# nivihelen99/NetFlow

Measured on AMD Instinct MI355X. Metric: device-resident payload GB/s checksummed, batched packets, 1/2/4/8 MI355X, higher is better.
Workload: dtype u16 one's-complement (u8 frames, u32 word sums); 1 GPU; C1: 1M x 1500 B IPv4+UDP, device-resident; packets_per_gpu=1048576, frame_align=128, frame_bytes_per_gpu=1572864000, parallelism=independent shards x1

## Files before the change

### netflow_amd/csrc/nfcs_api.hip

```cpp
#include <pthread.h>
#include <sched.h>
#include <stdio.h>
#include <stdlib.h>
#include <string.h>
#include <sys/mman.h>
#include <sys/syscall.h>
#include <unistd.h>

#include <algorithm>
#include <chrono>
#include <condition_variable>
#include <mutex>
#include <new>
#include <thread>
#include <type_traits>
#include <vector>

#include "nfcs_internal.h"
#include "nfcs_store_policy.h"

struct HostBlock {
    void* p = nullptr;
    size_t bytes = 0;
    bool mapped = false;
// ... 111 lines not shown
    nfcs_patch* h_patch[kSlots] = {nullptr, nullptr};
    uint64_t* d_digest = nullptr;
    hipEvent_t ev0 = nullptr, ev1 = nullptr;
    nfcs_patch* ws = nullptr;
    size_t ws_cap = 0;
    hipEvent_t ws_ev = nullptr;
    hipStream_t ws_stream = nullptr;
    bool ws_used = false;
    bool ws_own = false;
    uint32_t* eq_ws = nullptr;
    uint64_t eq_cap = 0;
    hipEvent_t eq_ev = nullptr;
    hipStream_t eq_stream = nullptr;
    bool eq_used = false;
    bool eq_own = false;
    uint32_t slot_bytes = 0;
    static constexpr int kObsSlots = 8;
    uint64_t* obs_host = nullptr;
    uint64_t* obs_dev = nullptr;
    struct ObsBurst { const void* desc; uint32_t n; uint64_t bytes; uint32_t gen; uint64_t used; };
    ObsBurst obs_burst[kObsSlots] = {};
    uint32_t obs_gen = 0;
    uint64_t obs_clock = 0;
    static constexpr int kDemRing = 64;
    uint32_t* dem_dev = nullptr;
    uint64_t* dem_host = nullptr;
    uint64_t* dem_host_dev = nullptr;
    uint32_t dem_gen = 0;
    struct DemCall { uint32_t gen, sampled; };
    DemCall dem_calls[kDemRing] = {};
// ... 68 lines not shown
            (void)hipGetLastError();
            return hipErrorOutOfMemory;
        }
        c->eq_cap = cap;
    } else if (c->eq_used && c->eq_stream != st) {
        hipError_t e = wait_eq_user(c, st);
        if (e != hipSuccess) return e;
    }
    return hipSuccess;
}
hipError_t release_eq(nfcs_ctx* c, hipStream_t st) {
    c->eq_stream = st;
    c->eq_used = true;
    c->eq_own = st == c->stream;
    return c->eq_own ? hipSuccess : hipEventRecord(c->eq_ev, st);
}

int hip_fail(hipError_t e) {
    g_last_hip = (int)e;
    return NFCS_EHIP;
}
#define NFCS_HIP(x)                              \
    do {                                         \
        hipError_t e_ = (x);                     \
        if (e_ != hipSuccess) return hip_fail(e_); \
    } while (0)

hipStream_t pick(nfcs_ctx* ctx, void* s) { return s ? (hipStream_t)s : ctx->stream; }

struct DeviceGuard {
// ... 617 lines not shown
}

template <class Launch>
int with_eq_scratch(nfcs_ctx* c, uint64_t words, hipStream_t st, Launch&& launch) {
    const hipError_t e = acquire_eq(c, words, st);
    if (e == hipErrorOutOfMemory) {
        (void)hipGetLastError();
        return NFCS_ENOMEM;
    }
    NFCS_HIP(e);
    NFCS_HIP(launch(c->eq_ws));
    NFCS_HIP(release_eq(c, st));
    return NFCS_OK;
}

}

extern "C" {

NFCS_API int nfcs_abi_version(void) { return NFCS_ABI_VERSION; }

NFCS_API const char* nfcs_strerror(int err) {
    switch (err) {
    case NFCS_OK: return "ok";
    case NFCS_EINVAL: return "invalid argument";
    case NFCS_EHIP: return "HIP runtime error";
    case NFCS_ENOMEM: return "out of memory";
    case NFCS_ENODEV: return "no gfx950 device";
    default: return "unknown error";
    }
// ... 11 lines not shown
    }
    DeviceGuard dg_(device);
    if (dg_.err != hipSuccess) return hip_fail(dg_.err);
    hipDeviceProp_t prop;
    NFCS_HIP(hipGetDeviceProperties(&prop, device));
    if (strncmp(prop.gcnArchName, "gfx950", 6) != 0) return NFCS_ENODEV;
    nfcs_ctx* c = new (std::nothrow) nfcs_ctx();
    if (!c) return NFCS_ENOMEM;
    c->di.device = device;
    c->di.cus = prop.multiProcessorCount;
    strncpy(c->di.arch, prop.gcnArchName, sizeof(c->di.arch) - 1);
    hipError_t e = hipStreamCreateWithFlags(&c->stream, hipStreamNonBlocking);
    if (e == hipSuccess) e = hipMalloc(&c->d_digest, sizeof(uint64_t));
    if (e == hipSuccess) e = hipEventCreateWithFlags(&c->ws_ev, hipEventDisableTiming);
    if (e == hipSuccess) e = hipEventCreateWithFlags(&c->eq_ev, hipEventDisableTiming);
    if (e == hipSuccess) e = hipEventCreate(&c->ev0);
    if (e == hipSuccess) e = hipEventCreate(&c->ev1);
    if (e == hipSuccess) e = hipHostMalloc((void**)&c->obs_host, nfcs_ctx::kObsSlots * sizeof(uint64_t), hipHostMallocMapped);
    if (e == hipSuccess) {
        for (int k = 0; k < nfcs_ctx::kObsSlots; ++k) c->obs_host[k] = 0;
        e = hipHostGetDevicePointer((void**)&c->obs_dev, c->obs_host, 0);
    }
    const size_t dem_bytes = 2u * nfcs::kDemandWords * nfcs::kDemandStrideWords * sizeof(uint32_t);
    if (e == hipSuccess) e = hipMalloc((void**)&c->dem_dev, dem_bytes);
    if (e == hipSuccess) e = hipMemset(c->dem_dev, 0, dem_bytes);
    if (e == hipSuccess) e = hipHostMalloc((void**)&c->dem_host, sizeof(uint64_t), hipHostMallocMapped);
    if (e == hipSuccess) {
        *c->dem_host = 0;
        e = hipHostGetDevicePointer((void**)&c->dem_host_dev, c->dem_host, 0);
    }
    if (e != hipSuccess) {
        nfcs_ctx_destroy(c);
        return hip_fail(e);
    }
    *out = c;
    return NFCS_OK;
}

NFCS_API int nfcs_ctx_destroy(nfcs_ctx* c) {
    if (!c) return NFCS_OK;
    DeviceGuard dg_(c->di.device);
    if (c->stream) (void)hipStreamSynchronize(c->stream);
    if (c->ws_used && !c->ws_own && c->ws_ev) (void)hipEventSynchronize(c->ws_ev);
    if (c->eq_used && !c->eq_own && c->eq_ev) (void)hipEventSynchronize(c->eq_ev);
    free_host_pipeline(c);
    if (c->d_digest) (void)hipFree(c->d_digest);
    if (c->eq_ws) (void)hipFree(c->eq_ws);
    if (c->eq_ev) (void)hipEventDestroy(c->eq_ev);
    if (c->ws) (void)hipFree(c->ws);
    if (c->ws_ev) (void)hipEventDestroy(c->ws_ev);
    if (c->ev0) (void)hipEventDestroy(c->ev0);
    if (c->ev1) (void)hipEventDestroy(c->ev1);
    if (c->stream) (void)hipStreamDestroy(c->stream);
    if (c->obs_host) (void)hipHostFree(c->obs_host);
    if (c->dem_host) (void)hipHostFree(c->dem_host);
    if (c->dem_dev) (void)hipFree(c->dem_dev);
    delete c;
    return NFCS_OK;
}

NFCS_API void* nfcs_ctx_stream(nfcs_ctx* c) { return c ? (void*)c->stream : nullptr; }

NFCS_API int nfcs_ctx_set_slot_bytes(nfcs_ctx* c, uint32_t bytes) {
// ... 635 lines not shown
}

NFCS_API int nfcs_egress_acl_device(nfcs_ctx* c, const nfcs_aclset* s, const uint8_t* d_arena, uint64_t arena_bytes,
                                    const nfcs_desc* d_desc, uint32_t n, uint32_t* d_port, uint8_t* d_action,
                                    uint32_t* d_rule, uint32_t* d_redirect, uint32_t* d_denied_pkts,
                                    uint64_t* d_denied_bytes, void* stream) {
    if (!usable(c, s)) return NFCS_EINVAL;
    if (!d_denied_pkts != !d_denied_bytes) return NFCS_EINVAL;
    DeviceGuard dg_(c->di.device);
    if (dg_.err != hipSuccess) return hip_fail(dg_.err);
    if (n == 0) return NFCS_OK;
    if (!d_arena || !d_desc || !d_port || !d_action || ((uintptr_t)d_arena & 15u)) return NFCS_EINVAL;
    if (((uintptr_t)d_port & 3u) || ((uintptr_t)d_rule & 3u) || ((uintptr_t)d_redirect & 3u) ||
        ((uintptr_t)d_denied_pkts & 3u) || ((uintptr_t)d_denied_bytes & 7u))
        return NFCS_EINVAL;
    NFCS_HIP(nfcs::launch_egress_acl(c->di, s->dev, d_arena, arena_bytes, d_desc, n, d_port, d_action, d_rule, d_redirect,
                                     d_denied_pkts, d_denied_bytes, pick(c, stream)));
    return NFCS_OK;
}

}

struct nfcs_txq {
    nfcs::TxqTables t;
    nfcs::TxqState h;
    nfcs_ctx* ctx = nullptr;
    int device = -1;
    uint8_t* d_blob = nullptr;
    uint8_t* d_ring = nullptr;
    size_t state_off = 0, state_bytes = 0;
    nfcs::TxqDev dev;
};

// ... 241 lines not shown
                                          uint32_t n, const uint8_t* d_action, const uint32_t* d_redirect,
                                          const uint8_t* d_rt_verdict, uint32_t* d_nh, uint32_t* d_l2_port,
                                          uint8_t* d_l2_verdict, uint8_t* d_class, uint8_t* d_bypass,
                                          nfcs_rx_stats* d_rx_stats, void* stream) {
    if (!usable(c, f)) return NFCS_EINVAL;
    DeviceGuard dg_(c->di.device);
    if (dg_.err != hipSuccess) return hip_fail(dg_.err);
    if (n == 0) return NFCS_OK;
    if (!d_arena || !d_desc || !d_rt_verdict || !d_nh || !d_l2_port || !d_l2_verdict || ((uintptr_t)d_arena & 15u))
        return NFCS_EINVAL;
    if (((uintptr_t)d_redirect & 3u) || ((uintptr_t)d_nh & 3u) || ((uintptr_t)d_l2_port & 3u) ||
        ((uintptr_t)d_rx_stats & 7u))
        return NFCS_EINVAL;
    const nfcs::DispatchArgs a{d_arena, arena_bytes, ingress_port, num_ports, n, d_desc, d_action, d_redirect,
                               d_rt_verdict, d_nh, d_l2_port, d_l2_verdict, d_class, d_bypass, d_rx_stats};
    NFCS_HIP(nfcs::launch_ingress_dispatch(c->di, f->dev, a, pick(c, stream)));
    return NFCS_OK;
}

NFCS_API int nfcs_egress_acl_items_host(const nfcs_aclset* s, const uint8_t* arena, uint64_t arena_bytes,
                                        const nfcs_desc* desc, uint32_t n, uint32_t* port, const uint32_t* item_src,
                                        const uint8_t* bypass, uint32_t n_src, uint8_t* action, uint32_t* rule,
                                        uint32_t* redirect, uint32_t* denied_pkts, uint64_t* denied_bytes) {
    if (!s || !s->committed || (!denied_pkts != !denied_bytes) || (!item_src != !bypass)) return NFCS_EINVAL;
    if (n == 0) return NFCS_OK;
    if (!arena || !desc || !port || !action) return NFCS_EINVAL;
    nfcs::aclset_egress(s->t, arena, arena_bytes, desc, n, port, action, rule, redirect, denied_pkts, denied_bytes,
                        item_src, bypass, n_src);
    return NFCS_OK;
}

NFCS_API int nfcs_egress_acl_items_device(nfcs_ctx* c, const nfcs_aclset* s, const uint8_t* d_arena, uint64_t arena_bytes,
                                          const nfcs_desc* d_desc, uint32_t n, uint32_t* d_port,
                                          const uint32_t* d_item_src, const uint8_t* d_bypass, uint32_t n_src,
                                          uint8_t* d_action, uint32_t* d_rule, uint32_t* d_redirect,
                                          uint32_t* d_denied_pkts, uint64_t* d_denied_bytes, void* stream) {
    if (!usable(c, s)) return NFCS_EINVAL;
    if ((!d_denied_pkts != !d_denied_bytes) || (!d_item_src != !d_bypass)) return NFCS_EINVAL;
    DeviceGuard dg_(c->di.device);
    if (dg_.err != hipSuccess) return hip_fail(dg_.err);
    if (n == 0) return NFCS_OK;
    if (!d_arena || !d_desc || !d_port || !d_action || ((uintptr_t)d_arena & 15u)) return NFCS_EINVAL;
    if (((uintptr_t)d_port & 3u) || ((uintptr_t)d_rule & 3u) || ((uintptr_t)d_redirect & 3u) ||
        ((uintptr_t)d_denied_pkts & 3u) || ((uintptr_t)d_denied_bytes & 7u) || ((uintptr_t)d_item_src & 3u))
        return NFCS_EINVAL;
    NFCS_HIP(nfcs::launch_egress_acl(c->di, s->dev, d_arena, arena_bytes, d_desc, n, d_port, d_action, d_rule, d_redirect,
                                     d_denied_pkts, d_denied_bytes, pick(c, stream), d_item_src, d_bypass, n_src));
    return NFCS_OK;
}

}

namespace {
struct RxWorkspace {
    uint64_t nh, eif, red, l2p, iport, ops, vlan, rt, st, act, l2v, byp, queue, eact, total;
};
RxWorkspace rx_workspace(uint32_t n, uint32_t cap) {
    uint64_t at = 0;
    auto part = [&at](uint64_t bytes) {
        const uint64_t o = at;
        at += (bytes + 15u) & ~15ull;
        return o;
    };
// ... 33 lines not shown
    if (!io->d_key_start || (tb->egress->dev.keys > 0 && !io->d_depth)) return NFCS_EINVAL;
    if (((uintptr_t)io->d_item_desc & 7u) || ((uintptr_t)io->d_item_port & 3u) || ((uintptr_t)io->d_item_src & 3u) ||
        ((uintptr_t)io->d_order & 3u) || ((uintptr_t)io->d_key_start & 3u) || ((uintptr_t)io->d_key_dropped & 3u) ||
        ((uintptr_t)io->d_depth & 3u) || ((uintptr_t)io->d_denied_pkts & 3u) || ((uintptr_t)io->d_denied_bytes & 7u) ||
        ((uintptr_t)io->d_rx_stats & 7u))
        return NFCS_EINVAL;
    hipStream_t st = pick(c, stream);
    uint8_t* ws = (uint8_t*)io->d_workspace;
    uint32_t *d_nh = (uint32_t*)(ws + w.nh), *d_eif = (uint32_t*)(ws + w.eif), *d_red = (uint32_t*)(ws + w.red);
    uint32_t *d_l2p = (uint32_t*)(ws + w.l2p), *d_iport = (uint32_t*)(ws + w.iport), *d_ops = (uint32_t*)(ws + w.ops);
    uint16_t* d_vlan = (uint16_t*)(ws + w.vlan);
    uint8_t *d_rt = ws + w.rt, *d_st = ws + w.st, *d_act = ws + w.act, *d_l2v = ws + w.l2v, *d_byp = ws + w.byp;
    uint8_t *d_queue = ws + w.queue, *d_eact = ws + w.eact;
    const bool acl = tb->ingress_acl != nullptr;
    const uint64_t frames = io->copy_base;
    NFCS_HIP(nfcs::launch_route_lookup(c->di, tb->fib->dev, io->d_arena, frames, io->d_desc, n, d_nh, d_eif, d_rt, st));
    if (acl)
        NFCS_HIP(nfcs::launch_acl_eval(c->di, tb->ingress_acl->dev, io->d_arena, frames, io->d_desc, n, d_act, nullptr,
                                       d_red, d_nh, st));
    NFCS_HIP(nfcs::launch_l2_lookup(c->di, tb->fdb->dev, io->ingress_port, io->d_arena, frames, io->d_desc, n, d_rt, d_l2p,
                                    d_l2v, d_vlan, nullptr, st));
    const nfcs::DispatchArgs da{io->d_arena, frames, io->ingress_port, io->num_ports, n, io->d_desc,
                                acl ? d_act : nullptr, acl ? d_red : nullptr, d_rt, d_nh, d_l2p, d_l2v, io->d_class, d_byp,
                                io->d_rx_stats};
    NFCS_HIP(nfcs::launch_ingress_dispatch(c->di, tb->fdb->dev, da, st));
    int rc = l3_forward_device(c, io->d_arena, frames, io->d_desc, d_nh, n, tb->fib->d_table, tb->fib->d_table_n, d_st, st);
    if (rc != NFCS_OK) return rc;
    const nfcs::FloodArgs fa{io->d_arena, io->arena_bytes, io->copy_base, io->copy_align, io->ingress_port, io->num_ports,
                             n, cap, io->d_desc, d_eif, d_st, d_l2p, d_l2v, d_vlan, io->d_item_desc, d_iport,
                             io->d_item_src, io->d_totals};
    rc = with_eq_scratch(c, nfcs::flood_scratch_words(n), st, [&](uint32_t* sc) {
        return nfcs::launch_flood_expand(c->di, tb->fdb->dev, fa, sc, st);
    });
    if (rc != NFCS_OK || cap == 0) return rc;
    NFCS_HIP(nfcs::launch_egress_plan(c->di, tb->egress->dev, io->d_arena, io->arena_bytes, io->d_item_desc, cap, nullptr,
                                      nullptr, d_iport, io->d_item_port, d_ops, d_queue, st));
    {
        const Shape sh = launch_shape(c, io->arena_bytes, io->d_item_desc, cap, kVlanRule);
        NFCS_HIP(nfcs::launch_vlan(c->di, io->d_arena, io->arena_bytes, io->d_item_desc, cap, d_ops, 0u, nullptr, 0u, nullptr,
                                   st, sh.mean, sh.obs, sh.bits));
    }
    if (tb->aclset)
        NFCS_HIP(nfcs::launch_egress_acl(c->di, tb->aclset->dev, io->d_arena, io->arena_bytes, io->d_item_desc, cap,
                                         io->d_item_port, d_eact, nullptr, nullptr, io->d_denied_pkts, io->d_denied_bytes,
                                         st, io->d_item_src, d_byp, n));
    rc = with_eq_scratch(c, nfcs::egress_scratch_words(cap, tb->egress->dev.keys), st, [&](uint32_t* sc) {
        return nfcs::launch_egress_enqueue(c->di, tb->egress->dev, io->d_item_port, d_queue, cap, io->d_depth, nullptr,
                                           io->d_order, io->d_key_start, io->d_key_dropped, sc, st);
    });
    if (rc != NFCS_OK) return rc;
    if (tb->txq)
        NFCS_HIP(nfcs::launch_txq_append(tb->txq->dev, io->d_order, io->d_key_start, io->d_depth, nullptr, nullptr, cap, st,
                                         io->handle_base));
    return NFCS_OK;
}

NFCS_API int nfcs_update_host(nfcs_ctx* c, uint8_t* h_arena, uint64_t arena_bytes,
                              const nfcs_desc* h_desc, uint32_t n, uint8_t* h_status,
                              uint32_t flags) {
    if (!c) return NFCS_EINVAL;
// ... 357 lines not shown
    if (!d_arena || !d_desc) return NFCS_EINVAL;
    NFCS_HIP(nfcs::launch_stale_every(d_arena, arena_bytes, d_desc, n, every, pick(c, stream)));
    return NFCS_OK;
}

NFCS_API int nfcs_digest_device(nfcs_ctx* c, const uint8_t* d_arena, uint64_t arena_bytes,
                                const nfcs_desc* d_desc, uint32_t n, uint64_t first,
                                uint64_t* h_digest, void* stream) {
    if (!c || !h_digest) return NFCS_EINVAL;
    DeviceGuard dg_(c->di.device);
    if (dg_.err != hipSuccess) return hip_fail(dg_.err);
    hipStream_t st = pick(c, stream);
    NFCS_HIP(hipMemsetAsync(c->d_digest, 0, sizeof(uint64_t), st));
    if (n) {
        if (!d_arena || !d_desc) return NFCS_EINVAL;
        NFCS_HIP(nfcs::launch_digest(c->di, d_arena, arena_bytes, d_desc, n, first, c->d_digest, st));
    }
    NFCS_HIP(hipMemcpyAsync(h_digest, c->d_digest, sizeof(uint64_t), hipMemcpyDeviceToHost, st));
    NFCS_HIP(hipStreamSynchronize(st));
    return NFCS_OK;
}

NFCS_API int nfcs_device_alloc(nfcs_ctx* c, size_t bytes, void** out) {
    if (!c || !out) return NFCS_EINVAL;
    DeviceGuard dg_(c->di.device);
    if (dg_.err != hipSuccess) return hip_fail(dg_.err);
    hipError_t e = hipMalloc(out, bytes ? bytes : 16);
    if (e == hipErrorOutOfMemory) { (void)hipGetLastError(); return NFCS_ENOMEM; }
    NFCS_HIP(e);
    return NFCS_OK;
}
// ... 178 lines not shown
```

### netflow_amd/csrc/nfcs_internal.h

```cpp
#pragma once

#include <hip/hip_runtime.h>
#include <stdint.h>

#include "nfcs.h"
#include "nfcs_acl.h"
#include "nfcs_aclset.h"
#include "nfcs_egress.h"
#include "nfcs_fdb.h"
#include "nfcs_fib.h"
#include "nfcs_icmp.h"
#include "nfcs_switch.h"
#include "nfcs_txq.h"

namespace nfcs {

constexpr int kWave = 64;
constexpr int kWavesPerBlock = 4;
constexpr int kBlock = kWave * kWavesPerBlock;

struct DevInfo {
    int device = 0;
    int cus = 256;
    char arch[64] = {0};
// ... 47 lines not shown
struct DemandReq {
    uint32_t* cur = nullptr;
    uint32_t* prev = nullptr;
    uint64_t* host = nullptr;
    uint32_t prev_gen = 0;
};
constexpr uint32_t kDemandSampleEvery = 64;
constexpr uint32_t kDemandWords = 64, kDemandStrideWords = 32;
constexpr uint32_t kDemandBlockPackets = 16;
inline uint32_t demand_sampled_one(uint32_t n) {
    const uint32_t span = kDemandSampleEvery * kDemandBlockPackets;
    const uint32_t rest = n % span;
    return n / span * kDemandBlockPackets + (rest < kDemandBlockPackets ? rest : kDemandBlockPackets);
}

hipError_t launch_update(const DevInfo& di, uint8_t* arena, uint64_t arena_bytes,
                         const nfcs_desc* desc, uint32_t n, uint32_t base16, uint8_t* status,
                         nfcs_patch* patch, nfcs_patch* ws, int form, hipStream_t stream,
                         uint64_t slot_bytes = 0, ObsReq obs = {}, DoneReq done = {}, DemandReq dem = {},
                         bool sparse = false);
uint32_t update_demand_sampled(uint64_t arena_bytes, uint32_t n, uint64_t slot_bytes, bool sparse);

hipError_t launch_l3_forward(const DevInfo& di, uint8_t* arena, uint64_t arena_bytes,
                             const nfcs_desc* desc, const uint32_t* nh, uint32_t n,
                             const nfcs_nexthop* table, uint32_t table_n, uint8_t* status,
                             nfcs_patch* ws, hipStream_t stream, uint64_t slot_bytes = 0,
                             ObsReq obs = {});

hipError_t launch_vlan(const DevInfo& di, uint8_t* arena, uint64_t arena_bytes, nfcs_desc* desc,
                       uint32_t n, const uint32_t* ops, uint32_t op_all, const uint32_t* caps,
// ... 26 lines not shown
};

hipError_t launch_acl_eval(const DevInfo& di, const AclDev& acl, const uint8_t* arena, uint64_t arena_bytes,
                           const nfcs_desc* desc, uint32_t n, uint8_t* action, uint32_t* rule, uint32_t* redirect,
                           uint32_t* nh, hipStream_t stream);

struct AclSetDev {
    const uint4* rec = nullptr;
    const uint2* act = nullptr;
    const uint2* bind = nullptr;
    uint32_t ports = 0, rules_padded = 0;
};

hipError_t launch_egress_acl(const DevInfo& di, const AclSetDev& set, const uint8_t* arena, uint64_t arena_bytes,
                             const nfcs_desc* desc, uint32_t n, uint32_t* port, uint8_t* action, uint32_t* rule,
                             uint32_t* redirect, uint32_t* denied_pkts, uint64_t* denied_bytes, hipStream_t stream,
                             const uint32_t* item_src = nullptr, const uint8_t* bypass = nullptr, uint32_t n_src = 0);

struct FdbDev {
    const uint4* slots = nullptr;
    uint32_t slot_mask = 0, max_probe = 0;
    const uint8_t* port_state = nullptr;
    const uint16_t* port_native = nullptr;
    const uint32_t* port_vlans = nullptr;
    uint32_t ports = 0;
    const uint32_t* vlan_ports = nullptr;
    uint32_t port_words = 0;
};

hipError_t launch_l2_lookup(const DevInfo& di, const FdbDev& fdb, uint32_t ingress, const uint8_t* arena,
                            uint64_t arena_bytes, const nfcs_desc* desc, uint32_t n, const uint8_t* rt_verdict,
// ... 8 lines not shown
struct DispatchArgs {
    const uint8_t* arena;
    uint64_t arena_bytes;
    uint32_t ingress, num_ports, n;
    const nfcs_desc* desc;
    const uint8_t* action;
    const uint32_t* redirect;
    const uint8_t* rt_verdict;
    uint32_t* nh;
    uint32_t* l2_port;
    uint8_t* l2_verdict;
    uint8_t* cls;
    uint8_t* bypass;
    nfcs_rx_stats* rx_stats;
};
hipError_t launch_ingress_dispatch(const DevInfo& di, const FdbDev& fdb, const DispatchArgs& a, hipStream_t stream);

hipError_t launch_egress_plan(const DevInfo& di, const EgressDev& eg, const uint8_t* arena, uint64_t arena_bytes,
                              const nfcs_desc* desc, uint32_t n, const uint32_t* l3_port, const uint8_t* fwd_status,
                              const uint32_t* l2_port, uint32_t* port, uint32_t* ops, uint8_t* queue,
                              hipStream_t stream);

constexpr uint32_t kEgTile = NFCS_EGRESS_TILE_PKTS;
static_assert(kEgTile % 64u == 0 && kEgTile >= 64u, "a tile is whole rounds of one wave");
inline uint64_t egress_scratch_words(uint32_t n, uint32_t keys) {
    const uint64_t tiles = ((uint64_t)n + kEgTile - 1u) / kEgTile;
    return tiles * keys + 2ull * keys;
}
hipError_t launch_egress_enqueue(const DevInfo& di, const EgressDev& eg, const uint32_t* port, const uint8_t* queue,
                                 uint32_t n, uint32_t* depth, uint8_t* result, uint32_t* order, uint32_t* key_start,
                                 uint32_t* key_dropped, uint32_t* scratch, hipStream_t stream);
// ... 63 lines not shown
    uint32_t* msg_port;
    uint32_t* msg_src;
    uint8_t* status;
    nfcs_icmp_totals* totals;
};
hipError_t launch_icmp_respond(const DevInfo& di, const IcmpView& icmp, const FibView& fib, const IcmpArgs& a,
                               uint32_t* scratch, hipStream_t stream);

hipError_t launch_stale_every(uint8_t* arena, uint64_t arena_bytes, const nfcs_desc* desc, uint32_t n,
                              uint32_t every, hipStream_t stream);
hipError_t launch_gen_config(const DevInfo& di, int config, uint64_t seed, uint64_t first,
                             uint32_t n, uint8_t* arena, uint64_t arena_bytes,
                             const nfcs_desc* desc, hipStream_t stream);

hipError_t launch_digest(const DevInfo& di, const uint8_t* arena, uint64_t arena_bytes,
                         const nfcs_desc* desc, uint32_t n, uint64_t first, uint64_t* d_out,
                         hipStream_t stream);

hipError_t launch_stream_read(const uint8_t* buf, uint64_t bytes, int form, unsigned long long* sink,
                              hipStream_t stream);

hipError_t launch_frames_read(const uint8_t* arena, uint64_t arena_bytes, const nfcs_desc* desc, uint32_t n,
                              unsigned long long* sink, hipStream_t stream);

uint32_t config_len(int config, uint64_t seed, uint64_t index);

}
```

### netflow_amd/csrc/nfcs_kernels.hip

```cpp
#include "nfcs_internal.h"

namespace nfcs {

#define DEV __device__ __forceinline__

DEV uint32_t rfl(uint32_t v) { return (uint32_t)__builtin_amdgcn_readfirstlane((int)v); }

DEV uint32_t xcd_block_n(uint32_t nblocks) {
    const uint32_t b = blockIdx.x, g8 = nblocks / 8u;
    return b < 8u * g8 ? (b % 8u) * g8 + b / 8u : b;
}
DEV uint32_t xcd_block() { return xcd_block_n(gridDim.x); }
DEV uint32_t bswap16(uint32_t x) { return ((x & 0xFFu) << 8) | ((x >> 8) & 0xFFu); }

__device__ __attribute__((aligned(4096))) uint4 g_zero_line[8];

DEV uint32_t comp(const uint4& v, uint32_t j) {
    const uint32_t m0 = 0u - (uint32_t)(j == 0), m1 = 0u - (uint32_t)(j == 1);
    const uint32_t m2 = 0u - (uint32_t)(j == 2), m3 = 0u - (uint32_t)(j == 3);
    return (v.x & m0) | (v.y & m1) | (v.z & m2) | (v.w & m3);
}


DEV uint4 put_byte(const uint4& v, uint32_t i, uint32_t b) {
// ... 1888 lines not shown
    }
}

hipError_t launch_acl_eval(const DevInfo& di, const AclDev& acl, const uint8_t* arena, uint64_t arena_bytes,
                           const nfcs_desc* desc, uint32_t n, uint8_t* action, uint32_t* rule, uint32_t* redirect,
                           uint32_t* nh, hipStream_t stream) {
    (void)di;
    if (n == 0) return hipSuccess;
    const uint32_t g = lane_blocks(n);
    const unsigned lds = kAclRowsBytes + acl.rules_padded * (unsigned)sizeof(AclRec);
    hipLaunchKernelGGL(acl_eval_kernel, dim3(g), dim3(kBlock), lds, stream, desc, n, g, arena, arena_bytes, acl, action,
                       rule, redirect, nh);
    return hipGetLastError();
}

constexpr uint32_t kEaSlotsBytes = kWavesPerBlock * 64u * 8u;
static_assert(kAclRowsBytes + kEaSlotsBytes + NFCS_ACL_MAX_RULES * sizeof(AclRec) < 64u * 1024u,
              "header rows + sum slots + rules stay under 64 KiB of dynamic LDS (no opt-in needed)");

__global__ __launch_bounds__(kBlock) void egress_acl_kernel(const nfcs_desc* __restrict__ desc, uint32_t n,
                                                            uint32_t nblocks, const uint8_t* __restrict__ arena,
                                                            uint64_t arena_bytes, uint32_t* __restrict__ port_io,
                                                            const AclSetDev set, uint8_t* __restrict__ action_out,
                                                            uint32_t* __restrict__ rule_out,
                                                            uint32_t* __restrict__ redirect_out,
                                                            uint32_t* __restrict__ denied_pkts,
                                                            unsigned long long* __restrict__ denied_bytes,
                                                            const uint32_t* __restrict__ item_src,
                                                            const uint8_t* __restrict__ bypass, uint32_t n_src) {
    extern __shared__ __attribute__((aligned(16))) uint8_t ea_lds[];
    const uint32_t lane = threadIdx.x & 63u, wave = threadIdx.x >> 6;
    const LanePkt lp = lane_pkt(desc, n, nblocks, arena_bytes);
    const uint64_t p0 = lp.p0, p = lp.p;
    const uint2 dl = lp.d;
    uint8_t* rows = ea_lds + wave * 64u * kFkRow;
    uint32_t port = NFCS_IF_NONE;
    if (p < n) port = port_io[p];
    const bool has_port = port != NFCS_IF_NONE;
    bool byp = false;
    if (item_src && has_port) {
        const uint32_t src = item_src[p];
        if (src < n_src) byp = bypass[src] != 0;
    }
    const bool live = lp.live && has_port && !byp;
    uint2 bind = make_uint2(0u, 0u);
    if (live && port < set.ports) bind = set.bind[port];
    const bool scan = bind.y != 0u;
    const uint32_t len = scan ? dl.y : 0u;
    const bool any = __builtin_amdgcn_ballot_w64(scan) != 0;
    uint4 c[8];
    if (any) hdr_rows_load(arena, dl.x, len, lane, c);
    stage_to_lds((uint4*)(ea_lds + kAclRowsBytes + kEaSlotsBytes), set.rec, set.rules_padded * 4u);
    __syncthreads();
    if (p0 >= n) return;
    uint32_t match = NFCS_ACL_NO_MATCH;
    if (any) {
        hdr_rows_store<kFkRow>(rows, lane, c);
        uint32_t key[8];
        acl_key_lds(rows + lane * kFkRow, arena, lp.off, len, key);
        const uint4* rec = (const uint4*)(ea_lds + kAclRowsBytes + kEaSlotsBytes);
        bool pending = scan;
        while (__builtin_amdgcn_ballot_w64(pending) != 0) {
            if (pending) {
                const uint32_t first = rfl(bind.x), end = first + rfl(bind.y);
                const bool mine = bind.x == first;
                for (uint32_t i = first; i < end; i += kAclGroup) {
                    if (__builtin_amdgcn_ballot_w64(mine && match == NFCS_ACL_NO_MATCH) == 0) break;
                    const uint32_t m = acl_scan_trip(rec, i, key);
                    match = (mine && match == NFCS_ACL_NO_MATCH) ? m : match;
// ... 5 lines not shown
    uint32_t action = !has_port ? NFCS_ACL_NO_PORT : byp ? NFCS_ACL_BYPASS : live ? NFCS_ACL_PERMIT : NFCS_ACL_BAD_DESC;
    uint32_t redirect = NFCS_IF_NONE, rule = NFCS_ACL_NO_MATCH;
    if (match != NFCS_ACL_NO_MATCH) {
        const uint2 a = set.act[match];
        action = a.x;
        redirect = a.y;
        rule = match - bind.x;
    }
    const bool denied = action == NFCS_ACL_DENY;
    if (p < n) {
        action_out[p] = (uint8_t)action;
        if (rule_out) rule_out[p] = rule;
        if (redirect_out) redirect_out[p] = redirect;
        if (denied || action == NFCS_ACL_BAD_DESC) port_io[p] = NFCS_IF_NONE;
    }
    if (denied_pkts && __builtin_amdgcn_ballot_w64(denied) != 0) {
        unsigned long long* slot = (unsigned long long*)(ea_lds + kAclRowsBytes) + wave * 64u;
        uint32_t lead = lane, cnt = 0;
        bool dp = denied;
        while (__builtin_amdgcn_ballot_w64(dp) != 0) {
            if (dp) {
                const uint32_t lp = rfl(port);
                if (port == lp) {
                    const uint64_t grp = __builtin_amdgcn_ballot_w64(true);
                    lead = (uint32_t)__builtin_ctzll(grp);
                    cnt = (uint32_t)__builtin_popcountll(grp);
                    dp = false;
                }
            }
        }
        const bool leader = denied && lead == lane;
        if (leader) slot[lane] = 0ull;
        __builtin_amdgcn_wave_barrier();
        if (denied) atomicAdd(&slot[lead], (unsigned long long)dl.y);
        __builtin_amdgcn_wave_barrier();
        if (leader) {
            atomicAdd(&denied_pkts[port], cnt);
            atomicAdd(&denied_bytes[port], slot[lane]);
        }
    }
}

hipError_t launch_egress_acl(const DevInfo& di, const AclSetDev& set, const uint8_t* arena, uint64_t arena_bytes,
                             const nfcs_desc* desc, uint32_t n, uint32_t* port, uint8_t* action, uint32_t* rule,
                             uint32_t* redirect, uint32_t* denied_pkts, uint64_t* denied_bytes, hipStream_t stream,
                             const uint32_t* item_src, const uint8_t* bypass, uint32_t n_src) {
    (void)di;
    if (n == 0) return hipSuccess;
    if (!item_src || !bypass) item_src = nullptr, bypass = nullptr, n_src = 0;
    const uint32_t g = lane_blocks(n);
    const unsigned lds = kAclRowsBytes + kEaSlotsBytes + set.rules_padded * (unsigned)sizeof(AclRec);
    hipLaunchKernelGGL(egress_acl_kernel, dim3(g), dim3(kBlock), lds, stream, desc, n, g, arena, arena_bytes, port, set,
                       action, rule, redirect, denied_pkts, (unsigned long long*)denied_bytes, item_src, bypass, n_src);
    return hipGetLastError();
}


DEV void fdb_step(const uint4& s, uint32_t k0, uint32_t k1, bool& search, bool& hit, uint32_t& port, uint32_t& flags) {
    const bool occ = (s.w & kFdbOccupied) != 0, m = search && occ && s.x == k0 && s.y == k1;
    port = m ? s.z : port;
    flags = m ? s.w : flags;
    hit = hit || m;
    search = search && !m && occ;
}

template <bool LEARN>
__global__ __launch_bounds__(kBlock) void l2_lookup_kernel(const nfcs_desc* __restrict__ desc, uint32_t n,
                                                           uint32_t nblocks, const uint8_t* __restrict__ arena,
// ... 141 lines not shown
                              const uint32_t* l2_port, uint32_t* port, uint32_t* ops, uint8_t* queue,
                              hipStream_t stream) {
    (void)di;
    if (n == 0) return hipSuccess;
    const uint32_t g = lane_blocks(n);
    hipLaunchKernelGGL(egress_plan_kernel, dim3(g), dim3(kBlock), 0, stream, desc, n, g, arena, arena_bytes, eg, l3_port,
                       fwd_status, l2_port, port, ops, queue);
    return hipGetLastError();
}

template <bool COUNT>
__global__ __launch_bounds__(kBlock) void ingress_dispatch_kernel(const nfcs_desc* __restrict__ desc, uint32_t n,
                                                                  uint32_t nblocks, const uint8_t* __restrict__ arena,
                                                                  uint64_t arena_bytes,
                                                                  const uint8_t* __restrict__ port_state, uint32_t ports,
                                                                  const DispatchArgs a) {
    __shared__ unsigned long long s_bytes[kWavesPerBlock];
    __shared__ uint32_t s_cnt[kWavesPerBlock];
    const uint32_t lane = threadIdx.x & 63u, wave = threadIdx.x >> 6;
    const LanePkt lp = lane_pkt(desc, n, nblocks, arena_bytes);
    if (!COUNT && lp.p0 >= n) return;
    const uint64_t p = lp.p, off = lp.off;
    const bool in = p < n, live = lp.live;
    uint32_t act = NFCS_ACL_PERMIT, red = NFCS_IF_NONE, rt = NFCS_RT_NOT_IPV4, l2v = NFCS_L2_SKIP;
    if (in) {
        if (a.action) act = a.action[p];
        if (a.redirect) red = a.redirect[p];
        rt = a.rt_verdict[p];
        l2v = a.l2_verdict[p];
    }
    const bool rx_up = a.ingress < ports && (port_state[a.ingress] & kSwLinkUp) != 0;
// ... 30 lines not shown
            by += ((unsigned long long)hi << 32) | lo;
        }
        if (lane == 0) {
            s_bytes[wave] = by;
            s_cnt[wave] = cnt;
        }
        __syncthreads();
        if (threadIdx.x == 0) {
            uint32_t tc = 0;
            unsigned long long tb = 0;
#pragma unroll
            for (int w = 0; w < kWavesPerBlock; ++w) {
                tc += s_cnt[w];
                tb += s_bytes[w];
            }
            unsigned long long* rx = (unsigned long long*)(a.rx_stats + a.ingress);
            if (tc & 0xFFFFu) atomicAdd(rx + 0, (unsigned long long)(tc & 0xFFFFu));
            if (tb) atomicAdd(rx + 1, tb);
            if (tc >> 16) atomicAdd(rx + 2, (unsigned long long)(tc >> 16));
        }
    }
}

hipError_t launch_ingress_dispatch(const DevInfo& di, const FdbDev& fdb, const DispatchArgs& a, hipStream_t stream) {
    (void)di;
    if (a.n == 0) return hipSuccess;
    const uint32_t g = lane_blocks(a.n);
    if (a.rx_stats)
        hipLaunchKernelGGL(ingress_dispatch_kernel<true>, dim3(g), dim3(kBlock), 0, stream, a.desc, a.n, g, a.arena,
                           a.arena_bytes, fdb.port_state, fdb.ports, a);
    else
        hipLaunchKernelGGL(ingress_dispatch_kernel<false>, dim3(g), dim3(kBlock), 0, stream, a.desc, a.n, g, a.arena,
                           a.arena_bytes, fdb.port_state, fdb.ports, a);
    return hipGetLastError();
}

constexpr uint32_t kEgRounds = kEgTile / 64u;
DEV uint32_t eg_class_at(const EgressDev& eg, const uint32_t* __restrict__ port, const uint8_t* __restrict__ queue,
                         uint64_t i, uint32_t n, uint32_t* key) {
    if (i >= n) return NFCS_EQ_SKIP;
    const uint32_t pt = port[i], q = queue[i];
    const bool has = pt < eg.ports;
    return egress_class(pt, q, has, eg_rec(eg, pt, has), key);
}

__global__ __launch_bounds__(64) void egress_hist_kernel(const uint32_t* __restrict__ port,
                                                         const uint8_t* __restrict__ queue, uint32_t n,
                                                         const EgressDev eg, uint32_t* __restrict__ hist) {
// ... 839 lines not shown
    NFCS_DPP_STEP(0x141)
    NFCS_DPP_STEP(0x140)
#undef NFCS_DPP_STEP
    uint64_t s = 0;
#pragma unroll
    for (int r = 0; r < 4; ++r)
        s += ((uint64_t)(uint32_t)__builtin_amdgcn_readlane((int)hi, 16 * r) << 32) |
             (uint32_t)__builtin_amdgcn_readlane((int)lo, 16 * r);
    return s;
}

__global__ __launch_bounds__(kBlock) void digest_kernel(const uint8_t* __restrict__ arena,
                                                        uint64_t arena_bytes,
                                                        const nfcs_desc* __restrict__ desc,
                                                        uint32_t n, uint64_t first,
                                                        unsigned long long* __restrict__ out) {
    const uint32_t lane = threadIdx.x & 63u;
    const uint32_t nw = gridDim.x * kWavesPerBlock;
    uint64_t wsum = 0;
    for (uint32_t p = blockIdx.x * kWavesPerBlock + rfl(threadIdx.x >> 6); p < n; p += nw) {
        const nfcs_desc d = desc[p];
        const uint64_t off = (uint64_t)d.off16 * 16u;
        const uint32_t len = d.len;
        if (off + (((uint64_t)len + 15) & ~15ull) > arena_bytes) continue;
        const uint4* src = (const uint4*)(arena + off);
        const uint32_t nch = (len + 15u) >> 4;
        uint64_t acc = 0;
        for (uint32_t c = lane; c < nch; c += 64u) {
            uint4 v = src[c];
            uint64_t lo = ((uint64_t)v.y << 32) | v.x, hi = ((uint64_t)v.w << 32) | v.z;
            const uint32_t o = c * 16u;
            if (o + 16 > len) {
                const uint32_t keep = len - o;
                if (keep < 8) { lo &= (1ull << (8 * keep)) - 1ull; hi = 0; }
                else if (keep == 8) { hi = 0; }
                else { hi &= (1ull << (8 * (keep - 8))) - 1ull; }
            }
            acc += mix64(lo ^ mix64(hi + (uint64_t)(c + 1) * kGolden));
        }
        const uint64_t h = mix64((uint64_t)len * 0xD6E8FEB86659FD93ull + wave_sum64(acc));
        wsum += mix64(h ^ ((first + p) * 0xA0761D6478BD642Full));
    }
    if (lane == 0 && wsum) atomicAdd(out, (unsigned long long)wsum);
}

hipError_t launch_digest(const DevInfo& di, const uint8_t* arena, uint64_t arena_bytes,
                         const nfcs_desc* desc, uint32_t n, uint64_t first, uint64_t* d_out,
                         hipStream_t stream) {
    if (n == 0) return hipSuccess;
    uint32_t grid = (n + kWavesPerBlock - 1) / kWavesPerBlock;
    if (grid > (uint32_t)di.cus * 8u) grid = (uint32_t)di.cus * 8u;
    hipLaunchKernelGGL(digest_kernel, dim3(grid), dim3(kBlock), 0, stream, arena, arena_bytes,
                       desc, n, first, (unsigned long long*)d_out);
    return hipGetLastError();
}


DEV TxqPort txq_port(const TxqDev& t, uint32_t p) {
    const uint4 r = t.port[p];
    return TxqPort{r.x, r.y, r.z, r.w};
}

DEV uint32_t txq_find_key(const uint32_t* __restrict__ start, uint32_t keys, uint32_t trips, uint32_t e) {
    uint32_t lo = 0, hi = keys + 1u;
    for (uint32_t s = 0; s < trips; ++s) {
        if (lo < hi) {
            const uint32_t mid = (lo + hi) >> 1;
            if (start[mid] > e) hi = mid;
// ... 175 lines not shown
```

Before: 6680 GB/s.

## Stripe global counter atomics across cache lines and fold them in a follow-up kernel

Replaces the single-address global atomics used for rx stats, denied-packet counters and the digest sum with striped per-stripe slots in a persistent scratch buffer, one cache line per stripe. A small fold kernel then sums the stripes, zeroes them and adds the totals to the user outputs. The egress ACL kernel also aggregates denied counts per port in a block-level LDS hash before issuing global atomics, and the digest kernel reduces per block before its atomic. The aim is less same-address atomic contention, at the cost of an extra kernel launch per call and scratch lifetime tracking across streams.

```diff
diff --git a/netflow_amd/csrc/nfcs_api.hip b/netflow_amd/csrc/nfcs_api.hip
--- a/netflow_amd/csrc/nfcs_api.hip
+++ b/netflow_amd/csrc/nfcs_api.hip
@@ -149,6 +149,11 @@
     hipStream_t eq_stream = nullptr;
     bool eq_used = false;
     bool eq_own = false;
+    uint64_t* ct_ws = nullptr;
+    hipEvent_t ct_ev = nullptr;
+    hipStream_t ct_stream = nullptr;
+    bool ct_used = false;
+    bool ct_own = false;
     uint32_t slot_bytes = 0;
     static constexpr int kObsSlots = 8;
     uint64_t* obs_host = nullptr;
@@ -247,6 +252,38 @@
     c->eq_used = true;
     c->eq_own = st == c->stream;
     return c->eq_own ? hipSuccess : hipEventRecord(c->eq_ev, st);
+}
+
+hipError_t acquire_ct(nfcs_ctx* c, hipStream_t st) {
+    if (!c->ct_ws) {
+        uint64_t* p = nullptr;
+        const size_t bytes = (size_t)nfcs::kCtSlots * sizeof(uint64_t);
+        hipError_t e = hipMalloc(&p, bytes);
+        if (e != hipSuccess) {
+            (void)hipGetLastError();
+            return hipErrorOutOfMemory;
+        }
+        e = hipMemset(p, 0, bytes);
+        if (e == hipSuccess) e = hipDeviceSynchronize();
+        if (e != hipSuccess) {
+            (void)hipFree(p);
+            return e;
+        }
+        c->ct_ws = p;
+    } else if (c->ct_used && c->ct_stream != st) {
+        if (c->ct_own) {
+            hipError_t e = hipEventRecord(c->ct_ev, c->stream);
+            if (e != hipSuccess) return e;
+        }
+        return hipStreamWaitEvent(st, c->ct_ev, 0);
+    }
+    return hipSuccess;
+}
+hipError_t release_ct(nfcs_ctx* c, hipStream_t st) {
+    c->ct_stream = st;
+    c->ct_used = true;
+    c->ct_own = st == c->stream;
+    return c->ct_own ? hipSuccess : hipEventRecord(c->ct_ev, st);
 }
 
 int hip_fail(hipError_t e) {
@@ -894,6 +931,20 @@
     return NFCS_OK;
 }
 
+template <class Launch>
+int with_ct_scratch(nfcs_ctx* c, bool counts, hipStream_t st, Launch&& launch) {
+    if (!counts) {
+        NFCS_HIP(launch((uint64_t*)nullptr));
+        return NFCS_OK;
+    }
+    const hipError_t e = acquire_ct(c, st);
+    if (e == hipErrorOutOfMemory) return NFCS_ENOMEM;
+    NFCS_HIP(e);
+    NFCS_HIP(launch(c->ct_ws));
+    NFCS_HIP(release_ct(c, st));
+    return NFCS_OK;
+}
+
 }
 
 extern "C" {
@@ -935,6 +986,7 @@
     if (e == hipSuccess) e = hipMalloc(&c->d_digest, sizeof(uint64_t));
     if (e == hipSuccess) e = hipEventCreateWithFlags(&c->ws_ev, hipEventDisableTiming);
     if (e == hipSuccess) e = hipEventCreateWithFlags(&c->eq_ev, hipEventDisableTiming);
+    if (e == hipSuccess) e = hipEventCreateWithFlags(&c->ct_ev, hipEventDisableTiming);
     if (e == hipSuccess) e = hipEventCreate(&c->ev0);
     if (e == hipSuccess) e = hipEventCreate(&c->ev1);
     if (e == hipSuccess) e = hipHostMalloc((void**)&c->obs_host, nfcs_ctx::kObsSlots * sizeof(uint64_t), hipHostMallocMapped);
@@ -964,10 +1016,13 @@
     if (c->stream) (void)hipStreamSynchronize(c->stream);
     if (c->ws_used && !c->ws_own && c->ws_ev) (void)hipEventSynchronize(c->ws_ev);
     if (c->eq_used && !c->eq_own && c->eq_ev) (void)hipEventSynchronize(c->eq_ev);
+    if (c->ct_used && !c->ct_own && c->ct_ev) (void)hipEventSynchronize(c->ct_ev);
     free_host_pipeline(c);
     if (c->d_digest) (void)hipFree(c->d_digest);
     if (c->eq_ws) (void)hipFree(c->eq_ws);
     if (c->eq_ev) (void)hipEventDestroy(c->eq_ev);
+    if (c->ct_ws) (void)hipFree(c->ct_ws);
+    if (c->ct_ev) (void)hipEventDestroy(c->ct_ev);
     if (c->ws) (void)hipFree(c->ws);
     if (c->ws_ev) (void)hipEventDestroy(c->ws_ev);
     if (c->ev0) (void)hipEventDestroy(c->ev0);
@@ -1633,9 +1688,11 @@
     if (((uintptr_t)d_port & 3u) || ((uintptr_t)d_rule & 3u) || ((uintptr_t)d_redirect & 3u) ||
         ((uintptr_t)d_denied_pkts & 3u) || ((uintptr_t)d_denied_bytes & 7u))
         return NFCS_EINVAL;
-    NFCS_HIP(nfcs::launch_egress_acl(c->di, s->dev, d_arena, arena_bytes, d_desc, n, d_port, d_action, d_rule, d_redirect,
-                                     d_denied_pkts, d_denied_bytes, pick(c, stream)));
-    return NFCS_OK;
+    hipStream_t st = pick(c, stream);
+    return with_ct_scratch(c, d_denied_pkts != nullptr, st, [&](uint64_t* ct) {
+        return nfcs::launch_egress_acl(c->di, s->dev, d_arena, arena_bytes, d_desc, n, d_port, d_action, d_rule, d_redirect,
+                                       d_denied_pkts, d_denied_bytes, ct, st);
+    });
 }
 
 }
@@ -1907,8 +1964,9 @@
         return NFCS_EINVAL;
     const nfcs::DispatchArgs a{d_arena, arena_bytes, ingress_port, num_ports, n, d_desc, d_action, d_redirect,
                                d_rt_verdict, d_nh, d_l2_port, d_l2_verdict, d_class, d_bypass, d_rx_stats};
-    NFCS_HIP(nfcs::launch_ingress_dispatch(c->di, f->dev, a, pick(c, stream)));
-    return NFCS_OK;
+    hipStream_t st = pick(c, stream);
+    return with_ct_scratch(c, d_rx_stats != nullptr, st,
+                           [&](uint64_t* ct) { return nfcs::launch_ingress_dispatch(c->di, f->dev, a, ct, st); });
 }
 
 NFCS_API int nfcs_egress_acl_items_host(const nfcs_aclset* s, const uint8_t* arena, uint64_t arena_bytes,
@@ -1937,9 +1995,11 @@
     if (((uintptr_t)d_port & 3u) || ((uintptr_t)d_rule & 3u) || ((uintptr_t)d_redirect & 3u) ||
         ((uintptr_t)d_denied_pkts & 3u) || ((uintptr_t)d_denied_bytes & 7u) || ((uintptr_t)d_item_src & 3u))
         return NFCS_EINVAL;
-    NFCS_HIP(nfcs::launch_egress_acl(c->di, s->dev, d_arena, arena_bytes, d_desc, n, d_port, d_action, d_rule, d_redirect,
-                                     d_denied_pkts, d_denied_bytes, pick(c, stream), d_item_src, d_bypass, n_src));
-    return NFCS_OK;
+    hipStream_t st = pick(c, stream);
+    return with_ct_scratch(c, d_denied_pkts != nullptr, st, [&](uint64_t* ct) {
+        return nfcs::launch_egress_acl(c->di, s->dev, d_arena, arena_bytes, d_desc, n, d_port, d_action, d_rule, d_redirect,
+                                       d_denied_pkts, d_denied_bytes, ct, st, d_item_src, d_bypass, n_src);
+    });
 }
 
 }
@@ -2003,6 +2063,12 @@
     uint8_t *d_queue = ws + w.queue, *d_eact = ws + w.eact;
     const bool acl = tb->ingress_acl != nullptr;
     const uint64_t frames = io->copy_base;
+    const bool counts = io->d_rx_stats || (cap > 0 && tb->aclset && io->d_denied_pkts);
+    if (counts) {
+        const hipError_t e = acquire_ct(c, st);
+        if (e == hipErrorOutOfMemory) return NFCS_ENOMEM;
+        NFCS_HIP(e);
+    }
     NFCS_HIP(nfcs::launch_route_lookup(c->di, tb->fib->dev, io->d_arena, frames, io->d_desc, n, d_nh, d_eif, d_rt, st));
     if (acl)
         NFCS_HIP(nfcs::launch_acl_eval(c->di, tb->ingress_acl->dev, io->d_arena, frames, io->d_desc, n, d_act, nullptr,
@@ -2012,7 +2078,8 @@
     const nfcs::DispatchArgs da{io->d_arena, frames, io->ingress_port, io->num_ports, n, io->d_desc,
                                 acl ? d_act : nullptr, acl ? d_red : nullptr, d_rt, d_nh, d_l2p, d_l2v, io->d_class, d_byp,
                                 io->d_rx_stats};
-    NFCS_HIP(nfcs::launch_ingress_dispatch(c->di, tb->fdb->dev, da, st));
+    NFCS_HIP(nfcs::launch_ingress_dispatch(c->di, tb->fdb->dev, da, c->ct_ws, st));
+    if (io->d_rx_stats) NFCS_HIP(release_ct(c, st));
     int rc = l3_forward_device(c, io->d_arena, frames, io->d_desc, d_nh, n, tb->fib->d_table, tb->fib->d_table_n, d_st, st);
     if (rc != NFCS_OK) return rc;
     const nfcs::FloodArgs fa{io->d_arena, io->arena_bytes, io->copy_base, io->copy_align, io->ingress_port, io->num_ports,
@@ -2029,10 +2096,12 @@
         NFCS_HIP(nfcs::launch_vlan(c->di, io->d_arena, io->arena_bytes, io->d_item_desc, cap, d_ops, 0u, nullptr, 0u, nullptr,
                                    st, sh.mean, sh.obs, sh.bits));
     }
-    if (tb->aclset)
+    if (tb->aclset) {
         NFCS_HIP(nfcs::launch_egress_acl(c->di, tb->aclset->dev, io->d_arena, io->arena_bytes, io->d_item_desc, cap,
                                          io->d_item_port, d_eact, nullptr, nullptr, io->d_denied_pkts, io->d_denied_bytes,
-                                         st, io->d_item_src, d_byp, n));
+                                         c->ct_ws, st, io->d_item_src, d_byp, n));
+        if (io->d_denied_pkts) NFCS_HIP(release_ct(c, st));
+    }
     rc = with_eq_scratch(c, nfcs::egress_scratch_words(cap, tb->egress->dev.keys), st, [&](uint32_t* sc) {
         return nfcs::launch_egress_enqueue(c->di, tb->egress->dev, io->d_item_port, d_queue, cap, io->d_depth, nullptr,
                                            io->d_order, io->d_key_start, io->d_key_dropped, sc, st);
@@ -2420,7 +2489,11 @@
     NFCS_HIP(hipMemsetAsync(c->d_digest, 0, sizeof(uint64_t), st));
     if (n) {
         if (!d_arena || !d_desc) return NFCS_EINVAL;
-        NFCS_HIP(nfcs::launch_digest(c->di, d_arena, arena_bytes, d_desc, n, first, c->d_digest, st));
+        const hipError_t e = acquire_ct(c, st);
+        if (e == hipErrorOutOfMemory) return NFCS_ENOMEM;
+        NFCS_HIP(e);
+        NFCS_HIP(nfcs::launch_digest(c->di, d_arena, arena_bytes, d_desc, n, first, c->d_digest, c->ct_ws, st));
+        NFCS_HIP(release_ct(c, st));
     }
     NFCS_HIP(hipMemcpyAsync(h_digest, c->d_digest, sizeof(uint64_t), hipMemcpyDeviceToHost, st));
     NFCS_HIP(hipStreamSynchronize(st));
diff --git a/netflow_amd/csrc/nfcs_internal.h b/netflow_amd/csrc/nfcs_internal.h
--- a/netflow_amd/csrc/nfcs_internal.h
+++ b/netflow_amd/csrc/nfcs_internal.h
@@ -85,6 +85,13 @@
     return n / span * kDemandBlockPackets + (rest < kDemandBlockPackets ? rest : kDemandBlockPackets);
 }
 
+constexpr uint32_t kCtStripes = 64;
+constexpr uint32_t kCtAclStripes = 16;
+constexpr uint32_t kCtLineSlots = 16;
+constexpr uint32_t kCtDispatchAt = 0, kCtDigestAt = kCtStripes * kCtLineSlots, kCtAclAt = 2u * kCtStripes * kCtLineSlots;
+constexpr uint32_t kCtSlots = kCtAclAt + kCtAclStripes * 2u * NFCS_L2_MAX_PORTS;
+inline uint32_t ct_acl_stride(uint32_t ports) { return (2u * ports + kCtLineSlots - 1u) & ~(kCtLineSlots - 1u); }
+
 hipError_t launch_update(const DevInfo& di, uint8_t* arena, uint64_t arena_bytes,
                          const nfcs_desc* desc, uint32_t n, uint32_t base16, uint8_t* status,
                          nfcs_patch* patch, nfcs_patch* ws, int form, hipStream_t stream,
@@ -141,7 +148,8 @@
 
 hipError_t launch_egress_acl(const DevInfo& di, const AclSetDev& set, const uint8_t* arena, uint64_t arena_bytes,
                              const nfcs_desc* desc, uint32_t n, uint32_t* port, uint8_t* action, uint32_t* rule,
-                             uint32_t* redirect, uint32_t* denied_pkts, uint64_t* denied_bytes, hipStream_t stream,
+                             uint32_t* redirect, uint32_t* denied_pkts, uint64_t* denied_bytes, uint64_t* ct,
+                             hipStream_t stream,
                              const uint32_t* item_src = nullptr, const uint8_t* bypass = nullptr, uint32_t n_src = 0);
 
 struct FdbDev {
@@ -180,7 +188,8 @@
     uint8_t* bypass;
     nfcs_rx_stats* rx_stats;
 };
-hipError_t launch_ingress_dispatch(const DevInfo& di, const FdbDev& fdb, const DispatchArgs& a, hipStream_t stream);
+hipError_t launch_ingress_dispatch(const DevInfo& di, const FdbDev& fdb, const DispatchArgs& a, uint64_t* ct,
+                                   hipStream_t stream);
 
 hipError_t launch_egress_plan(const DevInfo& di, const EgressDev& eg, const uint8_t* arena, uint64_t arena_bytes,
                               const nfcs_desc* desc, uint32_t n, const uint32_t* l3_port, const uint8_t* fwd_status,
@@ -274,7 +283,7 @@
                              const nfcs_desc* desc, hipStream_t stream);
 
 hipError_t launch_digest(const DevInfo& di, const uint8_t* arena, uint64_t arena_bytes,
-                         const nfcs_desc* desc, uint32_t n, uint64_t first, uint64_t* d_out,
+                         const nfcs_desc* desc, uint32_t n, uint64_t first, uint64_t* d_out, uint64_t* ct,
                          hipStream_t stream);
 
 hipError_t launch_stream_read(const uint8_t* buf, uint64_t bytes, int form, unsigned long long* sink,
diff --git a/netflow_amd/csrc/nfcs_kernels.hip b/netflow_amd/csrc/nfcs_kernels.hip
--- a/netflow_amd/csrc/nfcs_kernels.hip
+++ b/netflow_amd/csrc/nfcs_kernels.hip
@@ -1926,9 +1926,42 @@
     return hipGetLastError();
 }
 
-constexpr uint32_t kEaSlotsBytes = kWavesPerBlock * 64u * 8u;
+constexpr uint32_t kEaSlotsBytes = kWavesPerBlock * 64u * 8u + 16u;
+constexpr uint32_t kEaTableBytes = kBlock * 16u;
+static_assert(kEaTableBytes <= kAclRowsBytes, "the table lies in the header rows");
 static_assert(kAclRowsBytes + kEaSlotsBytes + NFCS_ACL_MAX_RULES * sizeof(AclRec) < 64u * 1024u,
               "header rows + sum slots + rules stay under 64 KiB of dynamic LDS (no opt-in needed)");
+
+template <uint32_t S>
+__global__ __launch_bounds__(kBlock) void counter_fold_kernel(unsigned long long* __restrict__ stripes, uint32_t stride,
+                                                              uint32_t slots, unsigned long long* __restrict__ out64,
+                                                              uint32_t* __restrict__ out32) {
+    const uint32_t j = blockIdx.x * kBlock + threadIdx.x;
+    if (j >= slots) return;
+    unsigned long long v[S], sum = 0;
+#pragma unroll
+    for (uint32_t k = 0; k < S; ++k)
+        v[k] = __hip_atomic_load(stripes + (uint64_t)k * stride + j, __ATOMIC_RELAXED, __HIP_MEMORY_SCOPE_AGENT);
+#pragma unroll
+    for (uint32_t k = 0; k < S; ++k) {
+        if (v[k]) __hip_atomic_store(stripes + (uint64_t)k * stride + j, 0ull, __ATOMIC_RELAXED, __HIP_MEMORY_SCOPE_AGENT);
+        sum += v[k];
+    }
+    if (!sum) return;
+    if (!out32)
+        atomicAdd(out64 + j, sum);
+    else if (j & 1u)
+        atomicAdd(out64 + (j >> 1), sum);
+    else
+        atomicAdd(out32 + (j >> 1), (uint32_t)sum);
+}
+
+template <uint32_t S>
+void launch_counter_fold(uint64_t* stripes, uint32_t stride, uint32_t slots, uint64_t* out64, uint32_t* out32,
+                         hipStream_t stream) {
+    hipLaunchKernelGGL(counter_fold_kernel<S>, dim3((slots + kBlock - 1u) / kBlock), dim3(kBlock), 0, stream,
+                       (unsigned long long*)stripes, stride, slots, (unsigned long long*)out64, out32);
+}
 
 __global__ __launch_bounds__(kBlock) void egress_acl_kernel(const nfcs_desc* __restrict__ desc, uint32_t n,
                                                             uint32_t nblocks, const uint8_t* __restrict__ arena,
@@ -1936,8 +1969,7 @@
                                                             const AclSetDev set, uint8_t* __restrict__ action_out,
                                                             uint32_t* __restrict__ rule_out,
                                                             uint32_t* __restrict__ redirect_out,
-                                                            uint32_t* __restrict__ denied_pkts,
-                                                            unsigned long long* __restrict__ denied_bytes,
+                                                            unsigned long long* __restrict__ ct, uint32_t ct_stride,
                                                             const uint32_t* __restrict__ item_src,
                                                             const uint8_t* __restrict__ bypass, uint32_t n_src) {
     extern __shared__ __attribute__((aligned(16))) uint8_t ea_lds[];
@@ -1963,8 +1995,10 @@
     uint4 c[8];
     if (any) hdr_rows_load(arena, dl.x, len, lane, c);
     stage_to_lds((uint4*)(ea_lds + kAclRowsBytes + kEaSlotsBytes), set.rec, set.rules_padded * 4u);
+    uint32_t* wg_denied = (uint32_t*)(ea_lds + kAclRowsBytes + kEaSlotsBytes - 16u);
+    if (ct && threadIdx.x == 0) *wg_denied = 0u;
     __syncthreads();
-    if (p0 >= n) return;
+    if (!ct && p0 >= n) return;
     uint32_t match = NFCS_ACL_NO_MATCH;
     if (any) {
         hdr_rows_store<kFkRow>(rows, lane, c);
@@ -2000,9 +2034,11 @@
         if (redirect_out) redirect_out[p] = redirect;
         if (denied || action == NFCS_ACL_BAD_DESC) port_io[p] = NFCS_IF_NONE;
     }
-    if (denied_pkts && __builtin_amdgcn_ballot_w64(denied) != 0) {
-        unsigned long long* slot = (unsigned long long*)(ea_lds + kAclRowsBytes) + wave * 64u;
-        uint32_t lead = lane, cnt = 0;
+    if (!ct) return;
+    unsigned long long* slot = (unsigned long long*)(ea_lds + kAclRowsBytes) + wave * 64u;
+    uint32_t lead = lane, cnt = 0;
+    bool leader = false;
+    if (__builtin_amdgcn_ballot_w64(denied) != 0) {
         bool dp = denied;
         while (__builtin_amdgcn_ballot_w64(dp) != 0) {
             if (dp) {
@@ -2015,29 +2051,57 @@
                 }
             }
         }
-        const bool leader = denied && lead == lane;
+        leader = denied && lead == lane;
         if (leader) slot[lane] = 0ull;
         __builtin_amdgcn_wave_barrier();
         if (denied) atomicAdd(&slot[lead], (unsigned long long)dl.y);
-        __builtin_amdgcn_wave_barrier();
-        if (leader) {
-            atomicAdd(&denied_pkts[port], cnt);
-            atomicAdd(&denied_bytes[port], slot[lane]);
-        }
+        if (lane == 0) *wg_denied = 1u;
+    }
+    __syncthreads();
+    if (*wg_denied == 0u) return;
+    uint32_t* t_port = (uint32_t*)ea_lds;
+    uint32_t* t_cnt = t_port + kBlock;
+    unsigned long long* t_bytes = (unsigned long long*)(t_cnt + kBlock);
+    t_port[threadIdx.x] = NFCS_IF_NONE;
+    t_cnt[threadIdx.x] = 0u;
+    t_bytes[threadIdx.x] = 0ull;
+    __syncthreads();
+    if (leader) {
+        uint32_t h = (port * 0x9E3779B1u) >> 24;
+        static_assert(kBlock == 256, "the hash keeps 8 bits");
+        for (uint32_t k = 0; k < kBlock; ++k, h = (h + 1u) & (kBlock - 1u)) {
+            const uint32_t was = atomicCAS(&t_port[h], (uint32_t)NFCS_IF_NONE, port);
+            if (was == NFCS_IF_NONE || was == port) {
+                atomicAdd(&t_cnt[h], cnt);
+                atomicAdd(&t_bytes[h], slot[lane]);
+                break;
+            }
+        }
+    }
+    __syncthreads();
+    const uint32_t tp = t_port[threadIdx.x];
+    if (tp != NFCS_IF_NONE) {
+        unsigned long long* to = ct + (uint64_t)(xcd_block_n(nblocks) % kCtAclStripes) * ct_stride + 2u * tp;
+        atomicAdd(to, (unsigned long long)t_cnt[threadIdx.x]);
+        atomicAdd(to + 1, t_bytes[threadIdx.x]);
     }
 }
 
 hipError_t launch_egress_acl(const DevInfo& di, const AclSetDev& set, const uint8_t* arena, uint64_t arena_bytes,
                              const nfcs_desc* desc, uint32_t n, uint32_t* port, uint8_t* action, uint32_t* rule,
-                             uint32_t* redirect, uint32_t* denied_pkts, uint64_t* denied_bytes, hipStream_t stream,
-                             const uint32_t* item_src, const uint8_t* bypass, uint32_t n_src) {
+                             uint32_t* redirect, uint32_t* denied_pkts, uint64_t* denied_bytes, uint64_t* ct,
+                             hipStream_t stream, const uint32_t* item_src, const uint8_t* bypass, uint32_t n_src) {
     (void)di;
     if (n == 0) return hipSuccess;
     if (!item_src || !bypass) item_src = nullptr, bypass = nullptr, n_src = 0;
+    if (denied_pkts && !ct) return hipErrorInvalidValue;
+    uint64_t* stripes = denied_pkts ? ct + kCtAclAt : nullptr;
+    const uint32_t stride = ct_acl_stride(set.ports);
     const uint32_t g = lane_blocks(n);
     const unsigned lds = kAclRowsBytes + kEaSlotsBytes + set.rules_padded * (unsigned)sizeof(AclRec);
     hipLaunchKernelGGL(egress_acl_kernel, dim3(g), dim3(kBlock), lds, stream, desc, n, g, arena, arena_bytes, port, set,
-                       action, rule, redirect, denied_pkts, (unsigned long long*)denied_bytes, item_src, bypass, n_src);
+                       action, rule, redirect, (unsigned long long*)stripes, stride, item_src, bypass, n_src);
+    if (stripes && set.ports) launch_counter_fold<kCtAclStripes>(stripes, stride, 2u * set.ports, denied_bytes, denied_pkts, stream);
     return hipGetLastError();
 }
 
@@ -2209,7 +2273,8 @@
                                                                   uint32_t nblocks, const uint8_t* __restrict__ arena,
                                                                   uint64_t arena_bytes,
                                                                   const uint8_t* __restrict__ port_state, uint32_t ports,
-                                                                  const DispatchArgs a) {
+                                                                  const DispatchArgs a,
+                                                                  unsigned long long* __restrict__ ct) {
     __shared__ unsigned long long s_bytes[kWavesPerBlock];
     __shared__ uint32_t s_cnt[kWavesPerBlock];
     const uint32_t lane = threadIdx.x & 63u, wave = threadIdx.x >> 6;
@@ -2270,7 +2335,7 @@
                 tc += s_cnt[w];
                 tb += s_bytes[w];
             }
-            unsigned long long* rx = (unsigned long long*)(a.rx_stats + a.ingress);
+            unsigned long long* rx = ct + (xcd_block_n(nblocks) % kCtStripes) * kCtLineSlots;
             if (tc & 0xFFFFu) atomicAdd(rx + 0, (unsigned long long)(tc & 0xFFFFu));
             if (tb) atomicAdd(rx + 1, tb);
             if (tc >> 16) atomicAdd(rx + 2, (unsigned long long)(tc >> 16));
@@ -2278,16 +2343,23 @@
     }
 }
 
-hipError_t launch_ingress_dispatch(const DevInfo& di, const FdbDev& fdb, const DispatchArgs& a, hipStream_t stream) {
+hipError_t launch_ingress_dispatch(const DevInfo& di, const FdbDev& fdb, const DispatchArgs& a, uint64_t* ct,
+                                   hipStream_t stream) {
     (void)di;
     if (a.n == 0) return hipSuccess;
     const uint32_t g = lane_blocks(a.n);
-    if (a.rx_stats)
+    if (a.rx_stats) {
+        if (!ct) return hipErrorInvalidValue;
+        static_assert(sizeof(nfcs_rx_stats) == 3u * sizeof(uint64_t), "rx_packets, rx_bytes, rx_drops: the three slots");
+        uint64_t* stripes = ct + kCtDispatchAt;
         hipLaunchKernelGGL(ingress_dispatch_kernel<true>, dim3(g), dim3(kBlock), 0, stream, a.desc, a.n, g, a.arena,
-                           a.arena_bytes, fdb.port_state, fdb.ports, a);
-    else
+                           a.arena_bytes, fdb.port_state, fdb.ports, a, (unsigned long long*)stripes);
+        if (a.ingress < fdb.ports)
+            launch_counter_fold<kCtStripes>(stripes, kCtLineSlots, 3u, (uint64_t*)(a.rx_stats + a.ingress), nullptr, stream);
+    } else {
         hipLaunchKernelGGL(ingress_dispatch_kernel<false>, dim3(g), dim3(kBlock), 0, stream, a.desc, a.n, g, a.arena,
-                           a.arena_bytes, fdb.port_state, fdb.ports, a);
+                           a.arena_bytes, fdb.port_state, fdb.ports, a, (unsigned long long*)nullptr);
+    }
     return hipGetLastError();
 }
 
@@ -3157,7 +3229,7 @@
                                                         uint64_t arena_bytes,
                                                         const nfcs_desc* __restrict__ desc,
                                                         uint32_t n, uint64_t first,
-                                                        unsigned long long* __restrict__ out) {
+                                                        unsigned long long* __restrict__ ct) {
     const uint32_t lane = threadIdx.x & 63u;
     const uint32_t nw = gridDim.x * kWavesPerBlock;
     uint64_t wsum = 0;
@@ -3184,17 +3256,28 @@
         const uint64_t h = mix64((uint64_t)len * 0xD6E8FEB86659FD93ull + wave_sum64(acc));
         wsum += mix64(h ^ ((first + p) * 0xA0761D6478BD642Full));
     }
-    if (lane == 0 && wsum) atomicAdd(out, (unsigned long long)wsum);
+    __shared__ unsigned long long s_sum[kWavesPerBlock];
+    if (lane == 0) s_sum[threadIdx.x >> 6] = wsum;
+    __syncthreads();
+    if (threadIdx.x == 0) {
+        unsigned long long t = 0;
+#pragma unroll
+        for (int w = 0; w < kWavesPerBlock; ++w) t += s_sum[w];
+        if (t) atomicAdd(ct + (blockIdx.x % kCtStripes) * kCtLineSlots, t);
+    }
 }
 
 hipError_t launch_digest(const DevInfo& di, const uint8_t* arena, uint64_t arena_bytes,
-                         const nfcs_desc* desc, uint32_t n, uint64_t first, uint64_t* d_out,
+                         const nfcs_desc* desc, uint32_t n, uint64_t first, uint64_t* d_out, uint64_t* ct,
                          hipStream_t stream) {
     if (n == 0) return hipSuccess;
+    if (!ct) return hipErrorInvalidValue;
     uint32_t grid = (n + kWavesPerBlock - 1) / kWavesPerBlock;
     if (grid > (uint32_t)di.cus * 8u) grid = (uint32_t)di.cus * 8u;
+    uint64_t* stripes = ct + kCtDigestAt;
     hipLaunchKernelGGL(digest_kernel, dim3(grid), dim3(kBlock), 0, stream, arena, arena_bytes,
-                       desc, n, first, (unsigned long long*)d_out);
+                       desc, n, first, (unsigned long long*)stripes);
+    launch_counter_fold<kCtStripes>(stripes, kCtLineSlots, 1u, d_out, nullptr, stream);
     return hipGetLastError();
 }
 
```

New measurement: 6857 GB/s (median of 6 runs). +2.7%, better.
